# OwshenNetwork/owshen

Measured on NVIDIA H100. Metric: groth16_withdraw_proofs_per_sec, higher is better.
Workload: dtype u256 (8x32-bit Montgomery limbs, integer)

## Files before the change

owshen_b200/api.py:

```python
import array
import bisect
import ctypes as C
import os
import secrets as _rand
import subprocess

_HERE = os.path.dirname(os.path.abspath(__file__))
_LIB_PATH = os.environ.get("OWSHEN_B200_LIB") or os.path.join(_HERE, "libowshen_b200.so")
_lib = None

FR_MODULUS = 21888242871839275222246405745257275088548364400416034343698204186575808495617
PROOF_BYTES = 256

OG_OK, OG_E_INVALID, OG_E_VERIFY = 0, -1, -6

NOTE_SUBGROUP_ORDER = 2736030358979909402780800718157159386076813972158567259200215660948447373041
NOTE_NOT_OWNED, NOTE_MALFORMED = 0xFFFFFFFF, 0xFFFFFFFE
NOTE_RECORD_BYTES, NOTE_PLAINTEXT_BYTES = 160, 128


class OwshenB200Error(RuntimeError):
    def __init__(self, code, detail=""):
        self.code = code
        msg = lib().og_strerror(code).decode() if _lib is not None else str(code)
# ... 275 lines not shown
        a, b = C.c_double(), C.c_double()
        _check(lib().og_imad_peak(self._h, C.byref(a), C.byref(b)), self)
        return a.value, b.value

    def mul_latency(self):
        a, b = C.c_double(), C.c_double()
        _check(lib().og_mul_latency(self._h, C.byref(a), C.byref(b)), self)
        return a.value, b.value

    def hybrid_probe(self) -> dict:
        r = (C.c_double * 4)()
        _check(lib().og_hybrid_probe(self._h, r), self)
        return {"fp64_products_52bit_alone": r[0], "imad_wide_chain_alone": r[1],
                "fp64_products_52bit_mixed": r[2], "imad_wide_chain_mixed": r[3]}

    def fp64_peak(self) -> float:
        v = C.c_double()
        _check(lib().og_fp64_peak(self._h, C.byref(v)), self)
        return v.value

    def int_pipe_peaks(self) -> dict:
        a, b, c = C.c_double(), C.c_double(), C.c_double()
        _check(lib().og_int_pipe_peaks(self._h, C.byref(a), C.byref(b), C.byref(c)), self)
        return {"imad_per_s": a.value, "imad_wide_per_s": b.value, "imad_wide_carry_chain_per_s": c.value}

    def field_op(self, field: str, op: str, a: bytes, b: bytes) -> bytes:
        _need(len(a) % 32 == 0 and len(b) == len(a), "field_op: a and b must be equally long multiples of 32 bytes")
        _need(field in ("fq", "fr") and op in ("mul", "add", "sub"), "field_op: unknown field or op")
        n = len(a) // 32
        out = C.create_string_buffer(32 * n)
        _check(lib().og_field_op(self._h, {"fq": 0, "fr": 1}[field], {"mul": 0, "add": 1, "sub": 2}[op], a, b, n, out), self)
        return out.raw

    FIELD_PROBE_OPS = {"g1": ("mul", "sqr", "sub", "dbl"),
                       "g2": ("mul_lazy", "sqr_lazy", "add_lazy", "sub_lazy", "canonical", "mul", "sqr", "is_zero_lazy")}

    def field_probe_raw(self, unit: str, op: str, a: bytes, b: bytes = None) -> bytes:
        _need(unit in self.FIELD_PROBE_OPS and op in self.FIELD_PROBE_OPS[unit], "field_probe_raw: unknown unit or op")
        eb = 32 if unit == "g1" else 64
        b = a if b is None else b
        _need(len(a) % eb == 0 and len(b) == len(a), f"field_probe_raw: a and b must be equally long multiples of {eb} bytes")
        n = len(a) // eb
        out = C.create_string_buffer(eb * n)
        _check(lib().og_field_probe_raw(self._h, unit == "g2", self.FIELD_PROBE_OPS[unit].index(op), a, b, n, out), self)
        return out.raw

    def msm_bucket_sums(self, curve: str, points: bytes, counts, entries, n_groups: int, nb: int, n_entries_max=None,
                        few_groups=False, buckets=False):
        _need(curve in ("g1", "g2"), "msm_bucket_sums: curve must be 'g1' or 'g2'")
        pb = 64 if curve == "g1" else 128
        _need(len(points) % pb == 0, f"msm_bucket_sums: points must be a multiple of {pb} bytes")
        def u32(xs):
            if not hasattr(xs, "astype"):
                return array.array("I", xs)
            a = array.array("I")
            a.frombytes(xs.astype("<u4").tobytes())
            return a
        cnt, ent = u32(counts), u32(entries)
        total = sum(cnt)
        _need(len(cnt) == n_groups * nb and len(ent) == total, "msm_bucket_sums: need n_groups * nb counts and sum(counts) entries")
        out = C.create_string_buffer(pb * n_groups)
        bk = C.create_string_buffer(pb * n_groups * nb) if buckets else None
        _check(lib().og_msm_bucket_sums(self._h, curve == "g2", points, len(points) // pb, C.c_void_p(cnt.buffer_info()[0]),
                                        C.c_void_p(ent.buffer_info()[0]) if total else None, n_groups, nb,
                                        total if n_entries_max is None else n_entries_max, int(few_groups), out, bk), self)
        return out.raw, (bk.raw if buckets else None)

    def mimc7_hash2(self, left: bytes, right: bytes) -> bytes:
        _need(len(left) % 32 == 0 and len(right) == len(left), "mimc7_hash2: left and right must be equally long multiples of 32 bytes")
        n = len(left) // 32
        out = C.create_string_buffer(32 * n)
# ... 666 lines not shown
```

owshen_b200/csrc/capi.cu:

```cuda
#include <stdlib.h>
#include <new>
#include "common.cuh"
#include "groth16.cuh"
#include "mimc.cuh"
#include "msm.cuh"
#include "ntt.cuh"
#include "withdraw_circuit.hpp"

using namespace og;

void* og_ctx::slot(int id, size_t bytes) {
    if (bytes == 0) bytes = 32;
    if (slot_cap[id] >= bytes) return slot_ptr[id];
    cudaDeviceSynchronize();
    if (slot_ptr[id]) cudaFree(slot_ptr[id]);
    slot_ptr[id] = nullptr; slot_cap[id] = 0;
    size_t cap = bytes + bytes / 8;
    cudaError_t e = cudaMalloc(&slot_ptr[id], cap);
    if (e != cudaSuccess) {
        e = cudaMalloc(&slot_ptr[id], bytes);
        cap = bytes;
    }
    if (e != cudaSuccess) {
        snprintf(err, sizeof(err), "slot %d: cudaMalloc(%zu) failed: %s", id, bytes, cudaGetErrorString(e));
// ... 1183 lines not shown
    uint64_t n_seg = 0;
    for (uint32_t k = 0; k < n_keys; k++)
        if (counts[k] > cap) n_seg += (counts[k] + (uint64_t)seg - 1) / seg;
    if (n_seg > msm_lvl_elems(n_groups, nb)) {
        snprintf(ctx->err, sizeof(ctx->err), "%llu heavy segments exceed the %llu segment sums of the level scratch", (unsigned long long)n_seg,
                 (unsigned long long)msm_lvl_elems(n_groups, nb));
        return OG_E_INVALID;
    }
    if (total && !entries) return OG_E_INVALID;
    for (uint64_t i = 0; i < total; i++)
        if ((entries[i] >> 1) >= n_points) { snprintf(ctx->err, sizeof(ctx->err), "entry %llu: point index out of range", (unsigned long long)i); return OG_E_INVALID; }
    const uint64_t pb = g2 ? 128 : 64;
    OG_SLOT(ctx, dp, uint8_t, S_IO_A, pb * n_points);
    OG_SLOT(ctx, de, uint32_t, S_IO_B, 4 * total);
    OG_SLOT(ctx, dc, uint32_t, S_IO_C, 4ull * n_keys);
    OG_SLOT(ctx, doff, uint32_t, S_IO_D, 4ull * (n_keys + 1ull));
    OG_SLOT(ctx, dtot, uint8_t, S_IO_E, pb * n_groups);
    uint8_t* dbk = nullptr;
    if (out_buckets) { dbk = (uint8_t*)ctx->slot(S_IO_F, pb * n_keys); if (!dbk) return OG_E_NOMEM; }
    OG_TRY(clear_flag(ctx));
    if (n_points) H2D(ctx, dp, points, pb * n_points);
    if (total) H2D(ctx, de, entries, 4 * total);
    H2D(ctx, dc, counts, 4ull * n_keys);
    H2D(ctx, doff, offsets.data(), 4ull * (n_keys + 1ull));
    if (g2) OG_TRY(msm_bucket_sums<Fq2>(ctx, dp, n_points, de, doff, dc, n_groups, nb, n_entries_max, few_groups != 0, dtot, dbk));
    else OG_TRY(msm_bucket_sums<Fq>(ctx, dp, n_points, de, doff, dc, n_groups, nb, n_entries_max, few_groups != 0, dtot, dbk));
    D2H(ctx, out_totals, dtot, pb * n_groups);
    if (out_buckets) D2H(ctx, out_buckets, dbk, pb * n_keys);
    return check_flag(ctx);
}

int32_t og_field_probe_raw(og_ctx* ctx, int32_t unit, int32_t op, const uint8_t* a, const uint8_t* b, uint64_t n, uint8_t* out) {
    OG_ENTER(ctx);
    if (unit < 0 || unit > 1 || op < 0 || op > (unit ? 7 : 3) || (n && (!a || !b || !out))) return OG_E_INVALID;
    if (n == 0) return OG_OK;
    const uint64_t eb = unit ? 64 : 32;
    OG_SLOT(ctx, da, uint8_t, S_IO_A, eb * n);
    OG_SLOT(ctx, db, uint8_t, S_IO_B, eb * n);
    OG_SLOT(ctx, dout, uint8_t, S_IO_C, eb * n);
    H2D(ctx, da, a, eb * n); H2D(ctx, db, b, eb * n);
    if (unit) OG_TRY(field_probe_raw<Fq2>(ctx, op, da, db, n, dout));
    else OG_TRY(field_probe_raw<Fq>(ctx, op, da, db, n, dout));
    D2H(ctx, out, dout, eb * n);
    OG_CUDA(ctx, cudaStreamSynchronize(ctx->stream));
    return OG_OK;
}

}
```

owshen_b200/csrc/ec.cuh:

```cuda
#pragma once
#include "fp.cuh"

namespace og {

template <class F>
struct Affine {
    F x, y;
    OG_HD static Affine inf() { return Affine{F::zero(), F::zero()}; }
    OG_HD bool is_inf() const { return x.is_zero() && y.is_zero(); }
    OG_HD Affine neg() const { return Affine{x, y.neg()}; }
    OG_HD bool operator==(const Affine& o) const { return x == o.x && y == o.y; }
};

template <class F>
struct XYZZ {
    F x, y, zz, zzz;

    OG_HD static XYZZ inf() { return XYZZ{F::one(), F::one(), F::zero(), F::zero()}; }
    OG_HD bool is_inf() const { return zz.is_zero(); }
    OG_HD static XYZZ from_affine(const Affine<F>& p) {
        if (p.is_inf()) return inf();
        return XYZZ{p.x, p.y, F::one(), F::one()};
    }
    OG_HD XYZZ neg() const { return XYZZ{x, y.neg(), zz, zzz}; }
// ... 77 lines not shown

    OG_HD static XYZZ mul(const Affine<F>& p, const uint32_t* k) {
        XYZZ acc = inf();
        for (int i = 255; i >= 0; i--) {
            acc = acc.dbl();
            if ((k[i >> 5] >> (i & 31)) & 1) acc.madd(p);
        }
        return acc;
    }
};

template <class Acc>
OG_HD bool g2_madd_lazy(const Acc& A, const Affine<Fq2>& q) {
    Fq2 p = Fq2::sub_lazy(fq2_mul_lazy(q.x, A.ld(2)), A.ld(0));
    Fq2 r = Fq2::sub_lazy(fq2_mul_lazy(q.y, A.ld(3)), A.ld(1));
    if (p.is_zero_lazy()) {
        if (!r.is_zero_lazy()) return false;
        XYZZ<Fq2> d = XYZZ<Fq2>::dbl_affine(q);
        A.st(0, d.x); A.st(1, d.y); A.st(2, d.zz); A.st(3, d.zzz);
        return true;
    }
    Fq2 pp = fq2_sqr_lazy(p);
    A.st(2, fq2_mul_lazy(A.ld(2), pp));
    Fq2 ppp = fq2_mul_lazy(p, pp);
    A.st(3, fq2_mul_lazy(A.ld(3), ppp));
    Fq2 q1 = fq2_mul_lazy(A.ld(0), pp);
    Fq2 x3 = Fq2::sub_lazy(Fq2::sub_lazy(fq2_sqr_lazy(r), ppp), Fq2::add_lazy(q1, q1));
    A.st(0, x3);
    Fq2 t = fq2_mul_lazy(A.ld(1), ppp);
    A.st(1, Fq2::sub_lazy(fq2_mul_lazy(r, Fq2::sub_lazy(q1, x3)), t));
    return true;
}

#if defined(__CUDACC__)
template <class F> __device__ __noinline__ void xyzz_add_ni(XYZZ<F>* a, const XYZZ<F>* b) { a->add(*b); }
template <class F> __device__ __noinline__ void xyzz_madd_ni(XYZZ<F>* a, const Affine<F>* b) { a->madd(*b); }
template <class F> __device__ __noinline__ void xyzz_dbl_ni(XYZZ<F>* a) { *a = a->dbl(); }
template <class F> __device__ __noinline__ void xyzz_to_affine_ni(Affine<F>* r, const XYZZ<F>* a) { *r = a->to_affine(); }
#endif

typedef Affine<Fq> G1Affine;
typedef Affine<Fq2> G2Affine;
typedef XYZZ<Fq> G1XYZZ;
typedef XYZZ<Fq2> G2XYZZ;

}
```

owshen_b200/csrc/fp.cuh:

```cuda
#pragma once
#include <stdint.h>
#include <string.h>

#if defined(__CUDACC__)
#define OG_HD __host__ __device__ __forceinline__
#else
#define OG_HD inline
#endif

namespace og {

struct CC { uint32_t c = 0; };

#if defined(__CUDA_ARCH__)
#define OG_ASM asm volatile
OG_HD uint32_t add_cc(uint32_t a, uint32_t b, CC&) { uint32_t r; OG_ASM("add.cc.u32 %0, %1, %2;" : "=r"(r) : "r"(a), "r"(b)); return r; }
OG_HD uint32_t addc_cc(uint32_t a, uint32_t b, CC&) { uint32_t r; OG_ASM("addc.cc.u32 %0, %1, %2;" : "=r"(r) : "r"(a), "r"(b)); return r; }
OG_HD uint32_t addc(uint32_t a, uint32_t b, CC&) { uint32_t r; OG_ASM("addc.u32 %0, %1, %2;" : "=r"(r) : "r"(a), "r"(b)); return r; }
OG_HD uint32_t sub_cc(uint32_t a, uint32_t b, CC&) { uint32_t r; OG_ASM("sub.cc.u32 %0, %1, %2;" : "=r"(r) : "r"(a), "r"(b)); return r; }
OG_HD uint32_t subc_cc(uint32_t a, uint32_t b, CC&) { uint32_t r; OG_ASM("subc.cc.u32 %0, %1, %2;" : "=r"(r) : "r"(a), "r"(b)); return r; }
OG_HD uint32_t subc(uint32_t a, uint32_t b, CC&) { uint32_t r; OG_ASM("subc.u32 %0, %1, %2;" : "=r"(r) : "r"(a), "r"(b)); return r; }
OG_HD uint32_t mad_lo_cc(uint32_t a, uint32_t b, uint32_t c, CC&) { uint32_t r; OG_ASM("mad.lo.cc.u32 %0, %1, %2, %3;" : "=r"(r) : "r"(a), "r"(b), "r"(c)); return r; }
OG_HD uint32_t madc_lo_cc(uint32_t a, uint32_t b, uint32_t c, CC&) { uint32_t r; OG_ASM("madc.lo.cc.u32 %0, %1, %2, %3;" : "=r"(r) : "r"(a), "r"(b), "r"(c)); return r; }
OG_HD uint32_t madc_hi_cc(uint32_t a, uint32_t b, uint32_t c, CC&) { uint32_t r; OG_ASM("madc.hi.cc.u32 %0, %1, %2, %3;" : "=r"(r) : "r"(a), "r"(b), "r"(c)); return r; }
// ... 28 lines not shown
    OG_HD static constexpr uint32_t one(int i) {
        constexpr uint32_t m[8] = {0xc58f0d9du, 0xd35d438du, 0xf5c70b3du, 0x0a78eb28u, 0x7879462cu, 0x666ea36fu, 0x9a07df2fu, 0x0e0a77c1u};
        return m[i];
    }
};
struct FrParams {
    static constexpr uint32_t INV = 0xefffffffu;
    OG_HD static constexpr uint32_t mod(int i) {
        constexpr uint32_t m[8] = {0xf0000001u, 0x43e1f593u, 0x79b97091u, 0x2833e848u, 0x8181585du, 0xb85045b6u, 0xe131a029u, 0x30644e72u};
        return m[i];
    }
    OG_HD static constexpr uint32_t r2(int i) {
        constexpr uint32_t m[8] = {0xae216da7u, 0x1bb8e645u, 0xe35c59e3u, 0x53fe3ab1u, 0x53bb8085u, 0x8c49833du, 0x7f4e44a5u, 0x0216d0b1u};
        return m[i];
    }
    OG_HD static constexpr uint32_t one(int i) {
        constexpr uint32_t m[8] = {0x4ffffffbu, 0xac96341cu, 0x9f60cd29u, 0x36fc7695u, 0x7879462eu, 0x666ea36fu, 0x9a07df2fu, 0x0e0a77c1u};
        return m[i];
    }
};

template <class P>
OG_HD void final_sub(uint32_t* r) {
    uint32_t t[8];
    CC cc;
    t[0] = sub_cc(r[0], P::mod(0), cc);
#pragma unroll
    for (int j = 1; j < 8; j++) t[j] = subc_cc(r[j], P::mod(j), cc);
    uint32_t borrow = subc(0u, 0u, cc);
#pragma unroll
    for (int j = 0; j < 8; j++) r[j] = borrow ? r[j] : t[j];
}

template <class P>
OG_HD void mont_row(uint32_t* E, uint32_t* O, const uint32_t* a, uint32_t bi, bool first) {
    CC cc;
    uint32_t orphan = 0;
    if (first) {
#pragma unroll
        for (int j = 0; j < 8; j += 2) {
            E[j] = mul_lo(a[j], bi);
            E[j + 1] = mul_hi(a[j], bi);
            O[j] = mul_lo(a[j + 1], bi);
            O[j + 1] = mul_hi(a[j + 1], bi);
        }
    } else {
        orphan = O[1];
        O[0] = mad_lo_cc(a[1], bi, O[2], cc);
        O[1] = madc_hi_cc(a[1], bi, O[3], cc);
#pragma unroll
        for (int j = 2; j < 6; j += 2) {
            O[j] = madc_lo_cc(a[j + 1], bi, O[j + 2], cc);
            O[j + 1] = madc_hi_cc(a[j + 1], bi, O[j + 3], cc);
        }
        O[6] = madc_lo_cc(a[7], bi, 0u, cc);
        O[7] = madc_hi(a[7], bi, 0u, cc);
        E[0] = mad_lo_cc(a[0], bi, E[0], cc);
        E[1] = madc_hi_cc(a[0], bi, E[1], cc);
#pragma unroll
        for (int j = 2; j < 8; j += 2) {
            E[j] = madc_lo_cc(a[j], bi, E[j], cc);
            E[j + 1] = madc_hi_cc(a[j], bi, E[j + 1], cc);
        }
        O[7] = addc(O[7], 0u, cc);
    }
    uint32_t s = add_cc(E[0], orphan, cc);
    uint32_t q = mul_lo(s, P::INV);
    O[0] = madc_lo_cc(P::mod(1), q, O[0], cc);
    O[1] = madc_hi_cc(P::mod(1), q, O[1], cc);
#pragma unroll
    for (int j = 2; j < 6; j += 2) {
        O[j] = madc_lo_cc(P::mod(j + 1), q, O[j], cc);
        O[j + 1] = madc_hi_cc(P::mod(j + 1), q, O[j + 1], cc);
    }
    O[6] = madc_lo_cc(P::mod(7), q, O[6], cc);
    O[7] = madc_hi(P::mod(7), q, O[7], cc);
    (void)add_cc(s, 0xffffffffu, cc);
    E[1] = madc_hi_cc(P::mod(0), q, E[1], cc);
#pragma unroll
    for (int j = 2; j < 8; j += 2) {
        E[j] = madc_lo_cc(P::mod(j), q, E[j], cc);
        E[j + 1] = madc_hi_cc(P::mod(j), q, E[j + 1], cc);
    }
    O[7] = addc(O[7], 0u, cc);
    E[0] = 0;
}

template <class P>
OG_HD constexpr uint32_t mod2(int i) { return (P::mod(i) << 1) | (i ? P::mod(i - 1) >> 31 : 0u); }

template <class P>
OG_HD void cond_sub_2p(uint32_t* r) {
    uint32_t t[8];
    CC cc;
    t[0] = sub_cc(r[0], mod2<P>(0), cc);
#pragma unroll
    for (int j = 1; j < 8; j++) t[j] = subc_cc(r[j], mod2<P>(j), cc);
    uint32_t borrow = subc(0u, 0u, cc);
#pragma unroll
    for (int j = 0; j < 8; j++) r[j] = borrow ? r[j] : t[j];
}

template <class P>
OG_HD void mont_mul_lazy(uint32_t* r, const uint32_t* a, const uint32_t* b) {
    uint32_t E[8], O[8];
    mont_row<P>(E, O, a, b[0], true);
    mont_row<P>(O, E, a, b[1], false);
    mont_row<P>(E, O, a, b[2], false);
    mont_row<P>(O, E, a, b[3], false);
    mont_row<P>(E, O, a, b[4], false);
    mont_row<P>(O, E, a, b[5], false);
    mont_row<P>(E, O, a, b[6], false);
    mont_row<P>(O, E, a, b[7], false);
    CC cc;
    r[0] = add_cc(E[0], O[1], cc);
#pragma unroll
    for (int j = 1; j < 7; j++) r[j] = addc_cc(E[j], O[j + 1], cc);
    r[7] = addc(E[7], 0u, cc);
}

template <class P>
OG_HD void mont_mul(uint32_t* r, const uint32_t* a, const uint32_t* b) {
    mont_mul_lazy<P>(r, a, b);
    final_sub<P>(r);
}


OG_HD void mul_wide(uint32_t* T, const uint32_t* a, const uint32_t* b) {
    uint32_t E[16], O[16];
#pragma unroll
    for (int k = 0; k < 16; k++) { E[k] = 0; O[k] = 0; }
    CC cc;
#pragma unroll
    for (int i = 0; i < 8; i++) {
        uint32_t* X = (i & 1) ? O : E;
        uint32_t* Y = (i & 1) ? E : O;
        const int x0 = (i & 1) ? i - 1 : i;
        const int y0 = (i & 1) ? i + 1 : i;
        X[x0] = mad_lo_cc(a[0], b[i], X[x0], cc);
        X[x0 + 1] = madc_hi_cc(a[0], b[i], X[x0 + 1], cc);
#pragma unroll
        for (int j = 2; j < 8; j += 2) {
            X[x0 + j] = madc_lo_cc(a[j], b[i], X[x0 + j], cc);
            X[x0 + j + 1] = madc_hi_cc(a[j], b[i], X[x0 + j + 1], cc);
        }
        if (x0 + 8 < 16) X[x0 + 8] = addc(X[x0 + 8], 0u, cc);
        Y[y0] = mad_lo_cc(a[1], b[i], Y[y0], cc);
        Y[y0 + 1] = madc_hi_cc(a[1], b[i], Y[y0 + 1], cc);
#pragma unroll
        for (int j = 2; j < 8; j += 2) {
            Y[y0 + j] = madc_lo_cc(a[j + 1], b[i], Y[y0 + j], cc);
            Y[y0 + j + 1] = madc_hi_cc(a[j + 1], b[i], Y[y0 + j + 1], cc);
        }
        if (y0 + 8 < 16) Y[y0 + 8] = addc(Y[y0 + 8], 0u, cc);
// ... 126 lines not shown
    OG_HD static Fp one() { Fp r;
#pragma unroll
        for (int i = 0; i < 8; i++) r.l[i] = P::one(i);
        return r; }
    OG_HD bool is_zero() const { uint32_t o = 0;
#pragma unroll
        for (int i = 0; i < 8; i++) o |= l[i];
        return o == 0; }
    OG_HD bool operator==(const Fp& b) const { uint32_t o = 0;
#pragma unroll
        for (int i = 0; i < 8; i++) o |= l[i] ^ b.l[i];
        return o == 0; }
    OG_HD bool operator!=(const Fp& b) const { return !(*this == b); }

    OG_HD friend Fp operator*(const Fp& a, const Fp& b) { Fp r; mont_mul<P>(r.l, a.l, b.l); return r; }
#if defined(OG_SQR_INTERLEAVED)
    OG_HD Fp sqr() const { Fp r; mont_mul<P>(r.l, l, l); return r; }
#else
    OG_HD Fp sqr() const { Fp r; uint32_t T[16]; sqr_wide(T, l); mont_reduce_wide<P>(r.l, T); return r; }
#endif

    OG_HD static Fp mul_lazy(const Fp& a, const Fp& b) { Fp r; mont_mul_lazy<P>(r.l, a.l, b.l); return r; }
    OG_HD Fp sqr_lazy() const { Fp r; uint32_t T[16]; sqr_wide(T, l); mont_reduce_wide_lazy<P>(r.l, T); return r; }
    OG_HD static Fp add_raw(const Fp& a, const Fp& b) {
        Fp r; CC cc;
        r.l[0] = add_cc(a.l[0], b.l[0], cc);
#pragma unroll
        for (int j = 1; j < 7; j++) r.l[j] = addc_cc(a.l[j], b.l[j], cc);
        r.l[7] = addc(a.l[7], b.l[7], cc);
        return r;
    }
    OG_HD Fp reduce_4p_to_2p() const { Fp r = *this; cond_sub_2p<P>(r.l); return r; }
    OG_HD Fp reduce_2p_to_p() const { Fp r = *this; final_sub<P>(r.l); return r; }

    OG_HD friend Fp operator+(const Fp& a, const Fp& b) {
        Fp r; CC cc;
        r.l[0] = add_cc(a.l[0], b.l[0], cc);
#pragma unroll
        for (int j = 1; j < 7; j++) r.l[j] = addc_cc(a.l[j], b.l[j], cc);
        r.l[7] = addc(a.l[7], b.l[7], cc);
        final_sub<P>(r.l);
        return r;
    }
    OG_HD friend Fp operator-(const Fp& a, const Fp& b) {
        Fp r; CC cc;
        r.l[0] = sub_cc(a.l[0], b.l[0], cc);
#pragma unroll
        for (int j = 1; j < 8; j++) r.l[j] = subc_cc(a.l[j], b.l[j], cc);
        uint32_t borrow = subc(0u, 0u, cc);
        r.l[0] = add_cc(r.l[0], P::mod(0) & borrow, cc);
#pragma unroll
        for (int j = 1; j < 7; j++) r.l[j] = addc_cc(r.l[j], P::mod(j) & borrow, cc);
        r.l[7] = addc(r.l[7], P::mod(7) & borrow, cc);
        return r;
    }
    OG_HD Fp neg() const { return zero() - *this; }
    OG_HD Fp dbl() const { return *this + *this; }

    OG_HD static Fp from_canonical(const uint32_t* c) {
        Fp t, r2;
#pragma unroll
        for (int i = 0; i < 8; i++) { t.l[i] = c[i]; r2.l[i] = P::r2(i); }
        return t * r2;
    }
    OG_HD void to_canonical(uint32_t* c) const {
        Fp o = zero(); o.l[0] = 1;
// ... 54 lines not shown
        T2[0] = sub_cc(T2[0], T0[0], cc);
        for (int j = 1; j < 15; j++) T2[j] = subc_cc(T2[j], T0[j], cc);
        T2[15] = subc(T2[15], T0[15], cc);
        T2[0] = sub_cc(T2[0], T1[0], cc);
        for (int j = 1; j < 15; j++) T2[j] = subc_cc(T2[j], T1[j], cc);
        T2[15] = subc(T2[15], T1[15], cc);
        T0[0] = sub_cc(T0[0], T1[0], cc);
        for (int j = 1; j < 15; j++) T0[j] = subc_cc(T0[j], T1[j], cc);
        T0[15] = subc(T0[15], T1[15], cc);
        T0[8] = add_cc(T0[8], FqParams::mod(0), cc);
        for (int j = 1; j < 7; j++) T0[8 + j] = addc_cc(T0[8 + j], FqParams::mod(j), cc);
        T0[15] = addc(T0[15], FqParams::mod(7), cc);
        Fq2 r;
        mont_reduce_wide<FqParams>(r.c0.l, T0);
        final_sub<FqParams>(r.c0.l);
        mont_reduce_wide<FqParams>(r.c1.l, T2);
        return r;
    }
    OG_HD static Fq2 sqr_inl(const Fq2& a) {
        Fq m = a.c0 * a.c1;
        return Fq2{(a.c0 + a.c1) * (a.c0 - a.c1), m + m};
    }
    OG_HD friend Fq2 operator*(const Fq2& a, const Fq2& b);
    OG_HD Fq2 sqr() const;
    OG_HD Fq2 neg() const { return Fq2{c0.neg(), c1.neg()}; }
    OG_HD Fq2 dbl() const { return Fq2{c0.dbl(), c1.dbl()}; }
    OG_HD Fq2 inv() const {
        Fq n = (c0.sqr() + c1.sqr()).inv();
        return Fq2{c0 * n, (c1 * n).neg()};
    }
    OG_HD Fq2 conj() const { return Fq2{c0, c1.neg()}; }
    OG_HD Fq2 mul_fq(const Fq& s) const { return Fq2{c0 * s, c1 * s}; }

    OG_HD static void add_lazy_fq(uint32_t* r, const uint32_t* a, const uint32_t* b) {
        CC cc;
        r[0] = add_cc(a[0], b[0], cc);
#pragma unroll
        for (int j = 1; j < 7; j++) r[j] = addc_cc(a[j], b[j], cc);
        r[7] = addc(a[7], b[7], cc);
        cond_sub_2p<FqParams>(r);
    }
    OG_HD static void sub_lazy_fq(uint32_t* r, const uint32_t* a, const uint32_t* b) {
        CC cc;
        r[0] = sub_cc(a[0], b[0], cc);
#pragma unroll
        for (int j = 1; j < 8; j++) r[j] = subc_cc(a[j], b[j], cc);
        uint32_t borrow = subc(0u, 0u, cc);
        r[0] = add_cc(r[0], mod2<FqParams>(0) & borrow, cc);
#pragma unroll
        for (int j = 1; j < 7; j++) r[j] = addc_cc(r[j], mod2<FqParams>(j) & borrow, cc);
        r[7] = addc(r[7], mod2<FqParams>(7) & borrow, cc);
    }
    OG_HD static void sub_raw_fq(uint32_t* r, const uint32_t* a, const uint32_t* b) {
        CC cc;
        r[0] = add_cc(a[0], mod2<FqParams>(0), cc);
#pragma unroll
        for (int j = 1; j < 7; j++) r[j] = addc_cc(a[j], mod2<FqParams>(j), cc);
        r[7] = addc(a[7], mod2<FqParams>(7), cc);
        r[0] = sub_cc(r[0], b[0], cc);
#pragma unroll
        for (int j = 1; j < 7; j++) r[j] = subc_cc(r[j], b[j], cc);
        r[7] = subc(r[7], b[7], cc);
    }
    OG_HD static bool is_zero_lazy_fq(const uint32_t* a) {
        uint32_t z = 0, q = 0;
#pragma unroll
        for (int j = 0; j < 8; j++) { z |= a[j]; q |= a[j] ^ FqParams::mod(j); }
        return z == 0 || q == 0;
    }
    OG_HD static Fq2 add_lazy(const Fq2& a, const Fq2& b) { Fq2 r; add_lazy_fq(r.c0.l, a.c0.l, b.c0.l); add_lazy_fq(r.c1.l, a.c1.l, b.c1.l); return r; }
    OG_HD static Fq2 sub_lazy(const Fq2& a, const Fq2& b) { Fq2 r; sub_lazy_fq(r.c0.l, a.c0.l, b.c0.l); sub_lazy_fq(r.c1.l, a.c1.l, b.c1.l); return r; }
    OG_HD bool is_zero_lazy() const { return is_zero_lazy_fq(c0.l) && is_zero_lazy_fq(c1.l); }
    OG_HD Fq2 canonical() const { Fq2 r = *this; final_sub<FqParams>(r.c0.l); final_sub<FqParams>(r.c1.l); return r; }

    OG_HD static Fq2 mul_lazy_inl(const Fq2& a, const Fq2& b) {
        uint32_t T0[16], T1[16], S[16];
        CC cc;
        mul_wide(T0, a.c0.l, b.c0.l);
        mul_wide(T1, a.c1.l, b.c1.l);
        S[0] = add_cc(T0[0], T1[0], cc);
#pragma unroll
        for (int j = 1; j < 15; j++) S[j] = addc_cc(T0[j], T1[j], cc);
        S[15] = addc(T0[15], T1[15], cc);
        T0[0] = sub_cc(T0[0], T1[0], cc);
#pragma unroll
        for (int j = 1; j < 15; j++) T0[j] = subc_cc(T0[j], T1[j], cc);
        T0[15] = subc(T0[15], T1[15], cc);
        T0[8] = add_cc(T0[8], FqParams::mod(0), cc);
#pragma unroll
        for (int j = 1; j < 7; j++) T0[8 + j] = addc_cc(T0[8 + j], FqParams::mod(j), cc);
        T0[15] = addc(T0[15], FqParams::mod(7), cc);
        Fq2 r;
        mont_reduce_wide_lazy<FqParams>(r.c0.l, T0);
        cond_sub_2p<FqParams>(r.c0.l);
        uint32_t sa[8], sb[8];
        sa[0] = add_cc(a.c0.l[0], a.c1.l[0], cc);
#pragma unroll
        for (int j = 1; j < 7; j++) sa[j] = addc_cc(a.c0.l[j], a.c1.l[j], cc);
        sa[7] = addc(a.c0.l[7], a.c1.l[7], cc);
        sb[0] = add_cc(b.c0.l[0], b.c1.l[0], cc);
#pragma unroll
        for (int j = 1; j < 7; j++) sb[j] = addc_cc(b.c0.l[j], b.c1.l[j], cc);
        sb[7] = addc(b.c0.l[7], b.c1.l[7], cc);
        mul_wide(T1, sa, sb);
        T1[0] = sub_cc(T1[0], S[0], cc);
#pragma unroll
        for (int j = 1; j < 15; j++) T1[j] = subc_cc(T1[j], S[j], cc);
        T1[15] = subc(T1[15], S[15], cc);
        mont_reduce_wide_lazy<FqParams>(r.c1.l, T1);
        cond_sub_2p<FqParams>(r.c1.l);
        return r;
    }
    OG_HD static Fq2 sqr_lazy_inl(const Fq2& a) {
        uint32_t T[16], u[8], v[8];
        Fq2 r;
        mul_wide(T, a.c0.l, a.c1.l);
        mont_reduce_wide_lazy<FqParams>(r.c1.l, T);
        add_lazy_fq(r.c1.l, r.c1.l, r.c1.l);
        add_lazy_fq(u, a.c0.l, a.c1.l);
        sub_raw_fq(v, a.c0.l, a.c1.l);
        mul_wide(T, u, v);
        mont_reduce_wide_lazy<FqParams>(r.c0.l, T);
        cond_sub_2p<FqParams>(r.c0.l);
        return r;
    }
};

#if defined(__CUDA_ARCH__) && defined(OG_FP_MUL_CALL)
static __device__ __noinline__ Fq2 fq2_mul_call(Fq2 a, Fq2 b) { return Fq2::mul_inl(a, b); }
static __device__ __noinline__ Fq2 fq2_sqr_call(Fq2 a) { return Fq2::sqr_inl(a); }
OG_HD Fq2 operator*(const Fq2& a, const Fq2& b) { return fq2_mul_call(a, b); }
OG_HD Fq2 Fq2::sqr() const { return fq2_sqr_call(*this); }
#else
OG_HD Fq2 operator*(const Fq2& a, const Fq2& b) { return Fq2::mul_inl(a, b); }
OG_HD Fq2 Fq2::sqr() const { return Fq2::sqr_inl(*this); }
#endif

#if defined(__CUDA_ARCH__) && defined(OG_FP_MUL_CALL)
static __device__ __noinline__ Fq2 fq2_mul_lazy_call(Fq2 a, Fq2 b) { return Fq2::mul_lazy_inl(a, b); }
static __device__ __noinline__ Fq2 fq2_sqr_lazy_call(Fq2 a) { return Fq2::sqr_lazy_inl(a); }
OG_HD Fq2 fq2_mul_lazy(const Fq2& a, const Fq2& b) { return fq2_mul_lazy_call(a, b); }
OG_HD Fq2 fq2_sqr_lazy(const Fq2& a) { return fq2_sqr_lazy_call(a); }
#else
OG_HD Fq2 fq2_mul_lazy(const Fq2& a, const Fq2& b) { return Fq2::mul_lazy_inl(a, b); }
OG_HD Fq2 fq2_sqr_lazy(const Fq2& a) { return Fq2::sqr_lazy_inl(a); }
#endif

}
```

owshen_b200/csrc/msm.cu:

```cuda
#include "msm.cuh"
#include "glv.cuh"
#include <stdlib.h>
#if !defined(OG_MSM_G1) && !defined(OG_MSM_G2)
#error "compile msm.cu with -DOG_MSM_G1 or -DOG_MSM_G2"
#endif

namespace og {

template <class F> struct FieldIO;
template <> struct FieldIO<Fq> {
    static constexpr int BYTES = 32;
    static __device__ __forceinline__ Fq load(const uint8_t* p, int* flag) { return load_canonical<Fq>(p, flag); }
    static __device__ __forceinline__ void store(uint8_t* p, const Fq& v) { store_canonical(p, v); }
};
template <> struct FieldIO<Fq2> {
    static constexpr int BYTES = 64;
    static __device__ __forceinline__ Fq2 load(const uint8_t* p, int* flag) {
        return Fq2{load_canonical<Fq>(p, flag), load_canonical<Fq>(p + 32, flag)};
    }
    static __device__ __forceinline__ void store(uint8_t* p, const Fq2& v) { store_canonical(p, v.c0); store_canonical(p + 32, v.c1); }
};

template <class F>
__global__ void __launch_bounds__(128) k_points_to_mont(const uint8_t* __restrict__ in, uint64_t n, Affine<F>* __restrict__ out, int* flag) {
    uint64_t i = (uint64_t)blockIdx.x * blockDim.x + threadIdx.x;
    if (i >= n) return;
    constexpr int B = FieldIO<F>::BYTES;
    const uint8_t* p = in + 2 * B * i;
    out[i] = Affine<F>{FieldIO<F>::load(p, flag), FieldIO<F>::load(p + B, flag)};
}
template <class F>
__global__ void __launch_bounds__(128) k_points_from_mont(const Affine<F>* __restrict__ in, uint64_t n, uint8_t* __restrict__ out) {
// ... 360 lines not shown
    }
    uint32_t base = t ? pair[t - 1] : 0;
    hist[2 * t] = base;
    hist[2 * t + 1] = base + a0;
    __syncthreads();
    for (uint32_t b = t; b < nb; b += 1024) {
        uint32_t pos = atomicAdd(&hist[ORDER_BINS - 1 - min(c[b], ORDER_BINS - 1)], 1u);
        perm[(size_t)g * nb + pos] = g * nb + b;
    }
}

template <class F>
__device__ __forceinline__ Affine<F> fetch_point(const Affine<F>* __restrict__ table, uint32_t e) {
    Affine<F> p = table[e >> 1];
    if (e & 1) p.y = p.y.neg();
    return p;
}

#ifdef OG_MSM_G1
struct SmAcc1 {
    uint4* base;
    __device__ __forceinline__ Fq ld(int coord) const {
        Fq v;
        uint4 a = base[(coord * 2 + 0) * 128], b = base[(coord * 2 + 1) * 128];
        v.l[0] = a.x; v.l[1] = a.y; v.l[2] = a.z; v.l[3] = a.w; v.l[4] = b.x; v.l[5] = b.y; v.l[6] = b.z; v.l[7] = b.w;
        return v;
    }
    __device__ __forceinline__ void st(int coord, const Fq& v) const {
        base[(coord * 2 + 0) * 128] = make_uint4(v.l[0], v.l[1], v.l[2], v.l[3]);
        base[(coord * 2 + 1) * 128] = make_uint4(v.l[4], v.l[5], v.l[6], v.l[7]);
    }
};

#ifndef OG_SQR_CALL
#define OG_SQR_CALL 1
#endif
#if OG_SQR_CALL
static __device__ __noinline__ Fq fq_sqr_call(Fq a) { return a.sqr(); }
#define OG_ACC_SQR(x) fq_sqr_call(x)
#else
#define OG_ACC_SQR(x) (x).sqr()
#endif
#if defined(OG_MUL_CALL) && OG_MUL_CALL
static __device__ __noinline__ Fq fq_mul_call(Fq a, Fq b) { return a * b; }
#define OG_ACC_MUL(x, y) fq_mul_call((x), (y))
#else
#define OG_ACC_MUL(x, y) ((x) * (y))
#endif
#ifndef OG_ACC1_MINB
#define OG_ACC1_MINB 8
#endif
__global__ void __launch_bounds__(128, OG_ACC1_MINB) k_bucket_acc_sm1(const Affine<Fq>* __restrict__ table, const uint32_t* __restrict__ sorted,
                                                        const uint32_t* __restrict__ offsets, const uint32_t* __restrict__ counts,
                                                        uint32_t n_keys, uint32_t cap, XYZZ<Fq>* __restrict__ buckets,
                                                        uint32_t* __restrict__ heavy, const uint32_t* __restrict__ perm) {
    __shared__ uint4 sm_acc[8 * 128];
    uint32_t slot_ = blockIdx.x * blockDim.x + threadIdx.x;
    if (slot_ >= n_keys) return;
    uint32_t key = perm[slot_];
    uint32_t cnt = counts[key], off = offsets[key];
    if (cnt > cap) {
        uint32_t slot = atomicAdd(heavy, 1u);
        heavy[1 + slot] = key;
        buckets[key] = XYZZ<Fq>::inf();
        return;
    }
    SmAcc1 A{sm_acc + threadIdx.x};
    bool inf = true;
    uint32_t e = cnt ? sorted[off] : 0;
    for (uint32_t k = 0; k < cnt; k++) {
        uint32_t en = k + 1 < cnt ? sorted[off + k + 1] : 0;
        Affine<Fq> q = fetch_point(table, e);
        e = en;
        if (q.is_inf()) continue;
        if (inf) { A.st(0, q.x); A.st(1, q.y); A.st(2, Fq::one()); A.st(3, Fq::one()); inf = false; continue; }
        Fq p = OG_ACC_MUL(q.x, A.ld(2)) - A.ld(0);
        Fq r = OG_ACC_MUL(q.y, A.ld(3)) - A.ld(1);
        if (p.is_zero()) {
            if (r.is_zero()) { XYZZ<Fq> d = XYZZ<Fq>::dbl_affine(q); A.st(0, d.x); A.st(1, d.y); A.st(2, d.zz); A.st(3, d.zzz); }
            else inf = true;
            continue;
        }
        Fq pp = OG_ACC_SQR(p);
        A.st(2, OG_ACC_MUL(A.ld(2), pp));
        Fq ppp = OG_ACC_MUL(p, pp);
        A.st(3, OG_ACC_MUL(A.ld(3), ppp));
        Fq q1 = OG_ACC_MUL(A.ld(0), pp);
        Fq x3 = OG_ACC_SQR(r) - ppp - q1.dbl();
        A.st(0, x3);
        A.st(1, OG_ACC_MUL(r, q1 - x3) - OG_ACC_MUL(A.ld(1), ppp));
    }
    buckets[key] = inf ? XYZZ<Fq>::inf() : XYZZ<Fq>{A.ld(0), A.ld(1), A.ld(2), A.ld(3)};
}

__global__ void __launch_bounds__(128, OG_ACC1_MINB) k_field_probe_g1(int32_t op, const Fq* __restrict__ a, const Fq* __restrict__ b, uint64_t n,
                                                        Fq* __restrict__ out) {
    uint64_t i = (uint64_t)blockIdx.x * blockDim.x + threadIdx.x;
    if (i >= n) return;
    const Fq x = a[i], y = b[i];
    out[i] = op == 0 ? OG_ACC_MUL(x, y) : op == 1 ? OG_ACC_SQR(x) : op == 2 ? x - y : x.dbl();
}
#endif

#ifdef OG_MSM_G2
struct SmAcc {
    uint4* base;
    __device__ __forceinline__ Fq2 ld(int coord) const {
        Fq2 v;
        uint4 a = base[(coord * 4 + 0) * 128], b = base[(coord * 4 + 1) * 128], c = base[(coord * 4 + 2) * 128], d = base[(coord * 4 + 3) * 128];
        v.c0.l[0] = a.x; v.c0.l[1] = a.y; v.c0.l[2] = a.z; v.c0.l[3] = a.w; v.c0.l[4] = b.x; v.c0.l[5] = b.y; v.c0.l[6] = b.z; v.c0.l[7] = b.w;
        v.c1.l[0] = c.x; v.c1.l[1] = c.y; v.c1.l[2] = c.z; v.c1.l[3] = c.w; v.c1.l[4] = d.x; v.c1.l[5] = d.y; v.c1.l[6] = d.z; v.c1.l[7] = d.w;
        return v;
    }
    __device__ __forceinline__ void st(int coord, const Fq2& v) const {
        base[(coord * 4 + 0) * 128] = make_uint4(v.c0.l[0], v.c0.l[1], v.c0.l[2], v.c0.l[3]);
        base[(coord * 4 + 1) * 128] = make_uint4(v.c0.l[4], v.c0.l[5], v.c0.l[6], v.c0.l[7]);
        base[(coord * 4 + 2) * 128] = make_uint4(v.c1.l[0], v.c1.l[1], v.c1.l[2], v.c1.l[3]);
        base[(coord * 4 + 3) * 128] = make_uint4(v.c1.l[4], v.c1.l[5], v.c1.l[6], v.c1.l[7]);
    }
};

#ifndef OG_ACC2_MINB
#define OG_ACC2_MINB 4
#endif
__global__ void __launch_bounds__(128, OG_ACC2_MINB) k_bucket_acc_sm(const Affine<Fq2>* __restrict__ table, const uint32_t* __restrict__ sorted,
                                                       const uint32_t* __restrict__ offsets, const uint32_t* __restrict__ counts,
                                                       uint32_t n_keys, uint32_t cap, XYZZ<Fq2>* __restrict__ buckets,
                                                       uint32_t* __restrict__ heavy, const uint32_t* __restrict__ perm) {
    __shared__ uint4 sm_acc[16 * 128];
    uint32_t slot_ = blockIdx.x * blockDim.x + threadIdx.x;
    if (slot_ >= n_keys) return;
    uint32_t key = perm[slot_];
    uint32_t cnt = counts[key], off = offsets[key];
// ... 704 lines not shown
```

Measured before the change: 2068.

## Use lazy-reduced field arithmetic and fused mul-sum in G1 bucket accumulation

The G1 bucket-accumulation kernel now keeps coordinates in the [0,2p) lazy range. It uses mul_lazy, sub_lazy, add_lazy and is_zero_lazy, and only canonicalizes when bucket results are written out. The final y-coordinate computation r*(q1-x3) - y*ppp becomes a single interleaved Montgomery multiply-sum with one reduction per row. This removes final subtractions and one full reduction pass per point addition. It adds correctness risk around the lazy-range bounds and the combined accumulation, and the diff also adds probe ops to test the new primitives.

```diff
diff --git a/owshen_b200/api.py b/owshen_b200/api.py
--- a/owshen_b200/api.py
+++ b/owshen_b200/api.py
@@ -331,11 +331,12 @@
         _check(lib().og_field_op(self._h, {"fq": 0, "fr": 1}[field], {"mul": 0, "add": 1, "sub": 2}[op], a, b, n, out), self)
         return out.raw
 
-    FIELD_PROBE_OPS = {"g1": ("mul", "sqr", "sub", "dbl"),
+    FIELD_PROBE_OPS = {"g1": ("mul", "sqr", "sub", "dbl", None, None, None, None,
+                              "mul_lazy", "sqr_lazy", "add_lazy", "sub_lazy", "canonical", "is_zero_lazy", "mul_sum_lazy"),
                        "g2": ("mul_lazy", "sqr_lazy", "add_lazy", "sub_lazy", "canonical", "mul", "sqr", "is_zero_lazy")}
 
     def field_probe_raw(self, unit: str, op: str, a: bytes, b: bytes = None) -> bytes:
-        _need(unit in self.FIELD_PROBE_OPS and op in self.FIELD_PROBE_OPS[unit], "field_probe_raw: unknown unit or op")
+        _need(unit in self.FIELD_PROBE_OPS and op is not None and op in self.FIELD_PROBE_OPS[unit], "field_probe_raw: unknown unit or op")
         eb = 32 if unit == "g1" else 64
         b = a if b is None else b
         _need(len(a) % eb == 0 and len(b) == len(a), f"field_probe_raw: a and b must be equally long multiples of {eb} bytes")
diff --git a/owshen_b200/csrc/capi.cu b/owshen_b200/csrc/capi.cu
--- a/owshen_b200/csrc/capi.cu
+++ b/owshen_b200/csrc/capi.cu
@@ -1239,7 +1239,8 @@
 
 int32_t og_field_probe_raw(og_ctx* ctx, int32_t unit, int32_t op, const uint8_t* a, const uint8_t* b, uint64_t n, uint8_t* out) {
     OG_ENTER(ctx);
-    if (unit < 0 || unit > 1 || op < 0 || op > (unit ? 7 : 3) || (n && (!a || !b || !out))) return OG_E_INVALID;
+    const bool op_ok = unit ? (op >= 0 && op <= 7) : ((op >= 0 && op <= 3) || (op >= 8 && op <= 14));
+    if (unit < 0 || unit > 1 || !op_ok || (n && (!a || !b || !out))) return OG_E_INVALID;
     if (n == 0) return OG_OK;
     const uint64_t eb = unit ? 64 : 32;
     OG_SLOT(ctx, da, uint8_t, S_IO_A, eb * n);
diff --git a/owshen_b200/csrc/ec.cuh b/owshen_b200/csrc/ec.cuh
--- a/owshen_b200/csrc/ec.cuh
+++ b/owshen_b200/csrc/ec.cuh
@@ -133,6 +133,27 @@
     return true;
 }
 
+template <class Acc>
+OG_HD bool g1_madd_lazy(const Acc& A, const Affine<Fq>& q) {
+    Fq p = Fq::sub_lazy(Fq::mul_lazy(q.x, A.ld(2)), A.ld(0));
+    Fq r = Fq::sub_lazy(Fq::mul_lazy(q.y, A.ld(3)), A.ld(1));
+    if (p.is_zero_lazy()) {
+        if (!r.is_zero_lazy()) return false;
+        XYZZ<Fq> d = XYZZ<Fq>::dbl_affine(q);
+        A.st(0, d.x); A.st(1, d.y); A.st(2, d.zz); A.st(3, d.zzz);
+        return true;
+    }
+    Fq pp = fq_sqr_lazy(p);
+    A.st(2, Fq::mul_lazy(A.ld(2), pp));
+    Fq ppp = Fq::mul_lazy(p, pp);
+    A.st(3, Fq::mul_lazy(A.ld(3), ppp));
+    Fq q1 = Fq::mul_lazy(A.ld(0), pp);
+    Fq x3 = Fq::sub_lazy(Fq::sub_lazy(fq_sqr_lazy(r), ppp), Fq::add_lazy(q1, q1));
+    A.st(0, x3);
+    A.st(1, Fq::mul_sum_lazy(r, Fq::sub_lazy(q1, x3), A.ld(1).neg_raw(), ppp));
+    return true;
+}
+
 #if defined(__CUDACC__)
 template <class F> __device__ __noinline__ void xyzz_add_ni(XYZZ<F>* a, const XYZZ<F>* b) { a->add(*b); }
 template <class F> __device__ __noinline__ void xyzz_madd_ni(XYZZ<F>* a, const Affine<F>* b) { a->madd(*b); }
diff --git a/owshen_b200/csrc/fp.cuh b/owshen_b200/csrc/fp.cuh
--- a/owshen_b200/csrc/fp.cuh
+++ b/owshen_b200/csrc/fp.cuh
@@ -84,8 +84,7 @@
     for (int j = 0; j < 8; j++) r[j] = borrow ? r[j] : t[j];
 }
 
-template <class P>
-OG_HD void mont_row(uint32_t* E, uint32_t* O, const uint32_t* a, uint32_t bi, bool first) {
+OG_HD uint32_t mont_row_mul(uint32_t* E, uint32_t* O, const uint32_t* a, uint32_t bi, bool first) {
     CC cc;
     uint32_t orphan = 0;
     if (first) {
@@ -116,6 +115,33 @@
         }
         O[7] = addc(O[7], 0u, cc);
     }
+    return orphan;
+}
+
+OG_HD void mont_row_addmul(uint32_t* E, uint32_t* O, const uint32_t* c, uint32_t di) {
+    CC cc;
+    O[0] = mad_lo_cc(c[1], di, O[0], cc);
+    O[1] = madc_hi_cc(c[1], di, O[1], cc);
+#pragma unroll
+    for (int j = 2; j < 6; j += 2) {
+        O[j] = madc_lo_cc(c[j + 1], di, O[j], cc);
+        O[j + 1] = madc_hi_cc(c[j + 1], di, O[j + 1], cc);
+    }
+    O[6] = madc_lo_cc(c[7], di, O[6], cc);
+    O[7] = madc_hi(c[7], di, O[7], cc);
+    E[0] = mad_lo_cc(c[0], di, E[0], cc);
+    E[1] = madc_hi_cc(c[0], di, E[1], cc);
+#pragma unroll
+    for (int j = 2; j < 8; j += 2) {
+        E[j] = madc_lo_cc(c[j], di, E[j], cc);
+        E[j + 1] = madc_hi_cc(c[j], di, E[j + 1], cc);
+    }
+    O[7] = addc(O[7], 0u, cc);
+}
+
+template <class P>
+OG_HD void mont_row_redc(uint32_t* E, uint32_t* O, uint32_t orphan) {
+    CC cc;
     uint32_t s = add_cc(E[0], orphan, cc);
     uint32_t q = mul_lo(s, P::INV);
     O[0] = madc_lo_cc(P::mod(1), q, O[0], cc);
@@ -139,6 +165,12 @@
 }
 
 template <class P>
+OG_HD void mont_row(uint32_t* E, uint32_t* O, const uint32_t* a, uint32_t bi, bool first) {
+    uint32_t orphan = mont_row_mul(E, O, a, bi, first);
+    mont_row_redc<P>(E, O, orphan);
+}
+
+template <class P>
 OG_HD constexpr uint32_t mod2(int i) { return (P::mod(i) << 1) | (i ? P::mod(i - 1) >> 31 : 0u); }
 
 template <class P>
@@ -151,6 +183,55 @@
     uint32_t borrow = subc(0u, 0u, cc);
 #pragma unroll
     for (int j = 0; j < 8; j++) r[j] = borrow ? r[j] : t[j];
+}
+
+template <class P>
+OG_HD void add_lazy_limbs(uint32_t* r, const uint32_t* a, const uint32_t* b) {
+    CC cc;
+    r[0] = add_cc(a[0], b[0], cc);
+#pragma unroll
+    for (int j = 1; j < 7; j++) r[j] = addc_cc(a[j], b[j], cc);
+    r[7] = addc(a[7], b[7], cc);
+    cond_sub_2p<P>(r);
+}
+template <class P>
+OG_HD void sub_lazy_limbs(uint32_t* r, const uint32_t* a, const uint32_t* b) {
+    CC cc;
+    r[0] = sub_cc(a[0], b[0], cc);
+#pragma unroll
+    for (int j = 1; j < 8; j++) r[j] = subc_cc(a[j], b[j], cc);
+    uint32_t borrow = subc(0u, 0u, cc);
+    r[0] = add_cc(r[0], mod2<P>(0) & borrow, cc);
+#pragma unroll
+    for (int j = 1; j < 7; j++) r[j] = addc_cc(r[j], mod2<P>(j) & borrow, cc);
+    r[7] = addc(r[7], mod2<P>(7) & borrow, cc);
+}
+template <class P>
+OG_HD void sub_raw_limbs(uint32_t* r, const uint32_t* a, const uint32_t* b) {
+    CC cc;
+    r[0] = add_cc(a[0], mod2<P>(0), cc);
+#pragma unroll
+    for (int j = 1; j < 7; j++) r[j] = addc_cc(a[j], mod2<P>(j), cc);
+    r[7] = addc(a[7], mod2<P>(7), cc);
+    r[0] = sub_cc(r[0], b[0], cc);
+#pragma unroll
+    for (int j = 1; j < 7; j++) r[j] = subc_cc(r[j], b[j], cc);
+    r[7] = subc(r[7], b[7], cc);
+}
+template <class P>
+OG_HD void neg_raw_limbs(uint32_t* r, const uint32_t* a) {
+    CC cc;
+    r[0] = sub_cc(mod2<P>(0), a[0], cc);
+#pragma unroll
+    for (int j = 1; j < 7; j++) r[j] = subc_cc(mod2<P>(j), a[j], cc);
+    r[7] = subc(mod2<P>(7), a[7], cc);
+}
+template <class P>
+OG_HD bool is_zero_lazy_limbs(const uint32_t* a) {
+    uint32_t z = 0, q = 0;
+#pragma unroll
+    for (int j = 0; j < 8; j++) { z |= a[j]; q |= a[j] ^ P::mod(j); }
+    return z == 0 || q == 0;
 }
 
 template <class P>
@@ -172,6 +253,24 @@
 }
 
 template <class P>
+OG_HD void mont_mul_sum_lazy(uint32_t* r, const uint32_t* a, const uint32_t* b, const uint32_t* c, const uint32_t* d) {
+    uint32_t E[8], O[8];
+#pragma unroll
+    for (int i = 0; i < 8; i++) {
+        uint32_t* X = (i & 1) ? O : E;
+        uint32_t* Y = (i & 1) ? E : O;
+        uint32_t orphan = mont_row_mul(X, Y, a, b[i], i == 0);
+        mont_row_addmul(X, Y, c, d[i]);
+        mont_row_redc<P>(X, Y, orphan);
+    }
+    CC cc;
+    r[0] = add_cc(E[0], O[1], cc);
+#pragma unroll
+    for (int j = 1; j < 7; j++) r[j] = addc_cc(E[j], O[j + 1], cc);
+    r[7] = addc(E[7], 0u, cc);
+}
+
+template <class P>
 OG_HD void mont_mul(uint32_t* r, const uint32_t* a, const uint32_t* b) {
     mont_mul_lazy<P>(r, a, b);
     final_sub<P>(r);
@@ -364,6 +463,14 @@
     }
     OG_HD Fp reduce_4p_to_2p() const { Fp r = *this; cond_sub_2p<P>(r.l); return r; }
     OG_HD Fp reduce_2p_to_p() const { Fp r = *this; final_sub<P>(r.l); return r; }
+    OG_HD static Fp add_lazy(const Fp& a, const Fp& b) { Fp r; add_lazy_limbs<P>(r.l, a.l, b.l); return r; }
+    OG_HD static Fp sub_lazy(const Fp& a, const Fp& b) { Fp r; sub_lazy_limbs<P>(r.l, a.l, b.l); return r; }
+    OG_HD Fp neg_raw() const { Fp r; neg_raw_limbs<P>(r.l, l); return r; }
+    OG_HD bool is_zero_lazy() const { return is_zero_lazy_limbs<P>(l); }
+    OG_HD Fp canonical() const { return reduce_2p_to_p(); }
+    OG_HD static Fp mul_sum_lazy(const Fp& a, const Fp& b, const Fp& c, const Fp& d) {
+        Fp r; mont_mul_sum_lazy<P>(r.l, a.l, b.l, c.l, d.l); cond_sub_2p<P>(r.l); return r;
+    }
 
     OG_HD friend Fp operator+(const Fp& a, const Fp& b) {
         Fp r; CC cc;
@@ -484,45 +591,9 @@
     OG_HD Fq2 conj() const { return Fq2{c0, c1.neg()}; }
     OG_HD Fq2 mul_fq(const Fq& s) const { return Fq2{c0 * s, c1 * s}; }
 
-    OG_HD static void add_lazy_fq(uint32_t* r, const uint32_t* a, const uint32_t* b) {
-        CC cc;
-        r[0] = add_cc(a[0], b[0], cc);
-#pragma unroll
-        for (int j = 1; j < 7; j++) r[j] = addc_cc(a[j], b[j], cc);
-        r[7] = addc(a[7], b[7], cc);
-        cond_sub_2p<FqParams>(r);
-    }
-    OG_HD static void sub_lazy_fq(uint32_t* r, const uint32_t* a, const uint32_t* b) {
-        CC cc;
-        r[0] = sub_cc(a[0], b[0], cc);
-#pragma unroll
-        for (int j = 1; j < 8; j++) r[j] = subc_cc(a[j], b[j], cc);
-        uint32_t borrow = subc(0u, 0u, cc);
-        r[0] = add_cc(r[0], mod2<FqParams>(0) & borrow, cc);
-#pragma unroll
-        for (int j = 1; j < 7; j++) r[j] = addc_cc(r[j], mod2<FqParams>(j) & borrow, cc);
-        r[7] = addc(r[7], mod2<FqParams>(7) & borrow, cc);
-    }
-    OG_HD static void sub_raw_fq(uint32_t* r, const uint32_t* a, const uint32_t* b) {
-        CC cc;
-        r[0] = add_cc(a[0], mod2<FqParams>(0), cc);
-#pragma unroll
-        for (int j = 1; j < 7; j++) r[j] = addc_cc(a[j], mod2<FqParams>(j), cc);
-        r[7] = addc(a[7], mod2<FqParams>(7), cc);
-        r[0] = sub_cc(r[0], b[0], cc);
-#pragma unroll
-        for (int j = 1; j < 7; j++) r[j] = subc_cc(r[j], b[j], cc);
-        r[7] = subc(r[7], b[7], cc);
-    }
-    OG_HD static bool is_zero_lazy_fq(const uint32_t* a) {
-        uint32_t z = 0, q = 0;
-#pragma unroll
-        for (int j = 0; j < 8; j++) { z |= a[j]; q |= a[j] ^ FqParams::mod(j); }
-        return z == 0 || q == 0;
-    }
-    OG_HD static Fq2 add_lazy(const Fq2& a, const Fq2& b) { Fq2 r; add_lazy_fq(r.c0.l, a.c0.l, b.c0.l); add_lazy_fq(r.c1.l, a.c1.l, b.c1.l); return r; }
-    OG_HD static Fq2 sub_lazy(const Fq2& a, const Fq2& b) { Fq2 r; sub_lazy_fq(r.c0.l, a.c0.l, b.c0.l); sub_lazy_fq(r.c1.l, a.c1.l, b.c1.l); return r; }
-    OG_HD bool is_zero_lazy() const { return is_zero_lazy_fq(c0.l) && is_zero_lazy_fq(c1.l); }
+    OG_HD static Fq2 add_lazy(const Fq2& a, const Fq2& b) { Fq2 r; add_lazy_limbs<FqParams>(r.c0.l, a.c0.l, b.c0.l); add_lazy_limbs<FqParams>(r.c1.l, a.c1.l, b.c1.l); return r; }
+    OG_HD static Fq2 sub_lazy(const Fq2& a, const Fq2& b) { Fq2 r; sub_lazy_limbs<FqParams>(r.c0.l, a.c0.l, b.c0.l); sub_lazy_limbs<FqParams>(r.c1.l, a.c1.l, b.c1.l); return r; }
+    OG_HD bool is_zero_lazy() const { return is_zero_lazy_limbs<FqParams>(c0.l) && is_zero_lazy_limbs<FqParams>(c1.l); }
     OG_HD Fq2 canonical() const { Fq2 r = *this; final_sub<FqParams>(r.c0.l); final_sub<FqParams>(r.c1.l); return r; }
 
     OG_HD static Fq2 mul_lazy_inl(const Fq2& a, const Fq2& b) {
@@ -568,9 +639,9 @@
         Fq2 r;
         mul_wide(T, a.c0.l, a.c1.l);
         mont_reduce_wide_lazy<FqParams>(r.c1.l, T);
-        add_lazy_fq(r.c1.l, r.c1.l, r.c1.l);
-        add_lazy_fq(u, a.c0.l, a.c1.l);
-        sub_raw_fq(v, a.c0.l, a.c1.l);
+        add_lazy_limbs<FqParams>(r.c1.l, r.c1.l, r.c1.l);
+        add_lazy_limbs<FqParams>(u, a.c0.l, a.c1.l);
+        sub_raw_limbs<FqParams>(v, a.c0.l, a.c1.l);
         mul_wide(T, u, v);
         mont_reduce_wide_lazy<FqParams>(r.c0.l, T);
         cond_sub_2p<FqParams>(r.c0.l);
@@ -598,4 +669,11 @@
 OG_HD Fq2 fq2_sqr_lazy(const Fq2& a) { return Fq2::sqr_lazy_inl(a); }
 #endif
 
-}
+#if defined(__CUDA_ARCH__) && defined(OG_FQ_SQR_CALL)
+static __device__ __noinline__ Fq fq_sqr_lazy_call(Fq a) { return a.sqr_lazy(); }
+OG_HD Fq fq_sqr_lazy(const Fq& a) { return fq_sqr_lazy_call(a); }
+#else
+OG_HD Fq fq_sqr_lazy(const Fq& a) { return a.sqr_lazy(); }
+#endif
+
+}
diff --git a/owshen_b200/csrc/msm.cu b/owshen_b200/csrc/msm.cu
--- a/owshen_b200/csrc/msm.cu
+++ b/owshen_b200/csrc/msm.cu
@@ -1,3 +1,6 @@
+#ifdef OG_MSM_G1
+#define OG_FQ_SQR_CALL
+#endif
 #include "msm.cuh"
 #include "glv.cuh"
 #include <stdlib.h>
@@ -424,21 +427,6 @@
     }
 };
 
-#ifndef OG_SQR_CALL
-#define OG_SQR_CALL 1
-#endif
-#if OG_SQR_CALL
-static __device__ __noinline__ Fq fq_sqr_call(Fq a) { return a.sqr(); }
-#define OG_ACC_SQR(x) fq_sqr_call(x)
-#else
-#define OG_ACC_SQR(x) (x).sqr()
-#endif
-#if defined(OG_MUL_CALL) && OG_MUL_CALL
-static __device__ __noinline__ Fq fq_mul_call(Fq a, Fq b) { return a * b; }
-#define OG_ACC_MUL(x, y) fq_mul_call((x), (y))
-#else
-#define OG_ACC_MUL(x, y) ((x) * (y))
-#endif
 #ifndef OG_ACC1_MINB
 #define OG_ACC1_MINB 8
 #endif
@@ -466,23 +454,9 @@
         e = en;
         if (q.is_inf()) continue;
         if (inf) { A.st(0, q.x); A.st(1, q.y); A.st(2, Fq::one()); A.st(3, Fq::one()); inf = false; continue; }
-        Fq p = OG_ACC_MUL(q.x, A.ld(2)) - A.ld(0);
-        Fq r = OG_ACC_MUL(q.y, A.ld(3)) - A.ld(1);
-        if (p.is_zero()) {
-            if (r.is_zero()) { XYZZ<Fq> d = XYZZ<Fq>::dbl_affine(q); A.st(0, d.x); A.st(1, d.y); A.st(2, d.zz); A.st(3, d.zzz); }
-            else inf = true;
-            continue;
-        }
-        Fq pp = OG_ACC_SQR(p);
-        A.st(2, OG_ACC_MUL(A.ld(2), pp));
-        Fq ppp = OG_ACC_MUL(p, pp);
-        A.st(3, OG_ACC_MUL(A.ld(3), ppp));
-        Fq q1 = OG_ACC_MUL(A.ld(0), pp);
-        Fq x3 = OG_ACC_SQR(r) - ppp - q1.dbl();
-        A.st(0, x3);
-        A.st(1, OG_ACC_MUL(r, q1 - x3) - OG_ACC_MUL(A.ld(1), ppp));
-    }
-    buckets[key] = inf ? XYZZ<Fq>::inf() : XYZZ<Fq>{A.ld(0), A.ld(1), A.ld(2), A.ld(3)};
+        if (!g1_madd_lazy(A, q)) inf = true;
+    }
+    buckets[key] = inf ? XYZZ<Fq>::inf() : XYZZ<Fq>{A.ld(0).canonical(), A.ld(1).canonical(), A.ld(2).canonical(), A.ld(3).canonical()};
 }
 
 __global__ void __launch_bounds__(128, OG_ACC1_MINB) k_field_probe_g1(int32_t op, const Fq* __restrict__ a, const Fq* __restrict__ b, uint64_t n,
@@ -490,7 +464,21 @@
     uint64_t i = (uint64_t)blockIdx.x * blockDim.x + threadIdx.x;
     if (i >= n) return;
     const Fq x = a[i], y = b[i];
-    out[i] = op == 0 ? OG_ACC_MUL(x, y) : op == 1 ? OG_ACC_SQR(x) : op == 2 ? x - y : x.dbl();
+    Fq z;
+    switch (op) {
+        case 0: z = x * y; break;
+        case 1: z = x.sqr(); break;
+        case 2: z = x - y; break;
+        case 3: z = x.dbl(); break;
+        case 8: z = Fq::mul_lazy(x, y); break;
+        case 9: z = fq_sqr_lazy(x); break;
+        case 10: z = Fq::add_lazy(x, y); break;
+        case 11: z = Fq::sub_lazy(x, y); break;
+        case 12: z = x.canonical(); break;
+        case 13: z = Fq::zero(); z.l[0] = x.is_zero_lazy() ? 1u : 0u; break;
+        default: { const Fq v = y.neg_raw(); z = Fq::mul_sum_lazy(x, x, v, v); break; }
+    }
+    out[i] = z;
 }
 #endif
 
```

New measurement: 2131 (median of 6 runs). +3.1%, better.
